# deryrahman/image-caption-emotion-indonesia

Hardware: AMD Instinct MI355X
Metric: images/sec (train step) + NLL loss match, batch=64 ResNet152+FactoredLSTM-512 (higher is better)
Workload: dtype f32 (trunk: operands as 2 f16 pieces each, 3 MFMA products per multiply, f32 accumulate; decoder: large products as 3 bf16 pieces per operand, 6 MFMA products per multiply, the rest f32 MFMA; the persistent LSTM kernel the trunk's split-f16 scheme)

## Files before the change

### image-caption-emotion-indonesia_amd/_lib.py

```python
import ctypes as C
import os

_HERE = os.path.dirname(os.path.abspath(__file__))
LIB_PATH = os.path.join(_HERE, "libcapnet_hip.so")

_f = C.POINTER(C.c_float)
_vp = C.c_void_p
_i = C.c_int
_l = C.c_long
_sz = C.c_size_t
_ip = C.POINTER(C.c_int)

SIGNATURES = {
    "capnet_last_error": (C.c_char_p, []),
    "capnet_abi_version": (_i, []),
    "capnet_sgemm": (_i, [_i, _i, _i, _i, _i, _vp, _l, _vp, _l, _vp, _l, _vp, _i, _i, _l, _l, _l,
                          _l, _i, _vp]),
    "capnet_sgemm_b3": (_i, [_i, _i, _i, _i, _i, _vp, _l, _vp, _l, _vp, _l, _vp, _i, _i, _l, _l, _l, _l, _vp, _sz, _vp]),
    "capnet_sgemm_b3_eligible": (_i, [_i, _i, _i, _i, _i, _vp, _l, _vp, _l, _vp, _l, _vp, _i, _l, _l, _l, _l]),
    "capnet_sgemm_splitk": (_i, [_i, _i, _i, _i, _i, _vp, _l, _vp, _l, _vp, _l, _vp, _i, _vp, _sz, _vp]),
    "capnet_sgemm_splitk_fused": (_i, [_i, _i, _i, _i, _i, _vp, _l, _vp, _l, _vp, _l, _vp, _i, _vp, _sz, _vp, _sz, _vp]),
    "capnet_colsum": (_i, [_vp, _l, _i, _i, _vp, _i, _vp]),
    "capnet_argmax_rows": (_i, [_vp, _i, _i, _i, _vp, _vp]),
    "capnet_resize_u8": (_i, [_vp, _i, _i, _vp, _vp, _i, _i, _vp, _vp, _i, _vp, _vp, _i, _vp]),
# ... 224 lines not shown
                                                                                                  _vp, _vp, _vp]),
    "capnet_beam_nbest": (_i, [_vp, _i, _i, _i, C.c_float, _vp, _vp, _vp, _vp, _vp]),
    "capnet_beam_nbest_traced": (_i, [_vp, _vp, _i, _i, _i, C.c_float, _vp, _vp, _vp, _vp, _vp, _vp]),
    "capnet_beam_decode_ws_beam_offset": (_sz, [_i] * 8),
    "capnet_att_beam_decode_alphas_ws_trace_offset": (_sz, [_i] * 11),
    "capnet_att_beam_decode_alphas_ws_hist_offset": (_sz, [_i] * 11),
    "capnet_alpha_gather": (_i, [_vp, _vp, _i, _i, _i, _i, _vp, _vp]),
    "capnet_lstm_wfrag_floats": (_sz, [_i]),
    "capnet_lstm_pack_wfrag": (_i, [_vp, _vp, _i, _i, _vp]),
    "capnet_lstm_step_fused": (_i, [_vp, _vp, _vp, _l, _vp, _vp, _vp, _i, _i, _i, _vp]),
    "capnet_lstm_step_fused_stamped": (_i, [_vp, _vp, _vp, _l, _vp, _vp, _vp, _i, _i, _vp, _vp]),
    "capnet_lstm_step_fused_supported": (_i, [_i, _i]),
    "capnet_lstm_persist_supported": (_i, [_i, _i]),
    "capnet_lstm_persist_w_floats": (_sz, []),
    "capnet_lstm_persist_ctl_ints": (_sz, []),
    "capnet_lstm_persist_pack": (_i, [_vp, _vp, _i, _vp]),
    "capnet_lstm_persist_run": (_i, [_vp, _vp, _vp, _vp, _ip, _i, _i, _i, _i, _i, _vp, _vp, _vp, _vp]),
    "capnet_xent_fwd": (_i, [_vp, _l, _i, _i, _vp, _vp, _vp, _vp, _vp, _vp]),
    "capnet_xent_bwd": (_i, [_vp, _l, _i, _i, _vp, _vp, _vp, _vp, _l, _vp]),
    "capnet_att_loss_fwd": (_i, [_vp, _vp, _i, _i, _i, C.c_float, _vp, _vp, _vp]),
    "capnet_att_loss_bwd": (_i, [_vp, _vp, _i, _i, _i, C.c_float, _vp, _vp]),
    "capnet_policy_xent_fwd": (_i, [_vp, _l, _i, _i, _vp, _vp, _i, _ip, _i, _vp, _vp, _vp, _vp, _vp, _vp]),
    "capnet_policy_xent_bwd": (_i, [_vp, _l, _i, _i, _vp, _vp, _vp, _i, _ip, _i, _vp, _vp, _l, _vp]),
    "capnet_bleu_rows": (_i, [_vp, _l, _i, _i, C.c_longlong, C.c_longlong, _i, _vp, _vp, _i, _i, _i, C.POINTER(C.c_double), _i,
                              _vp, _vp, _vp]),
    "capnet_cider_rows": (_i, [_vp, _l, _i, _i, C.c_longlong, C.c_longlong, _i, _vp, _vp, _vp, _i, _i, _i, C.POINTER(_vp),
                               C.POINTER(_vp), _ip, C.c_double, C.c_double, _vp, _vp, _vp, _vp]),
    "capnet_clamp_adam": (_i, [_i, C.POINTER(_vp), C.POINTER(_vp), C.POINTER(_vp),
                               C.POINTER(_vp), C.POINTER(_l), _ip, C.c_float, C.c_float,
                               C.c_float, C.c_float, C.c_float, _i, _vp, _vp]),
    "capnet_lstm_persist_set_mode": (_i, [_i]),
    "capnet_att_set_chain_mode": (_i, [_i]),
    "capnet_lstm_pointwise_bwd": (_i, [_vp, _vp, _vp, _vp, _vp, _vp, _i, _i, _i, _vp]),
    "capnet_conv1x1_fwd_areg": (_i, [_vp, _vp, _i, _vp, _vp, _vp, _i, _vp, _vp, _l, _i, _i, _i, _vp]),
    "capnet_trunk_set_timing": (_i, [_vp, _i]),
    "capnet_trunk_time_next_pass": (_i, [_vp]),
    "capnet_trunk_collect_timing": (_i, [_vp, C.POINTER(C.c_double), C.POINTER(_l),
                                         C.POINTER(C.c_double)]),
    "capnet_packed_targets": (_i, [_vp, _i, _i, _ip, _vp, _vp]),
    "capnet_fused_block_weight_words": (_sz, [_i, _i, _i]),
    "capnet_fused_block_pack": (_i, [_vp, _vp, _i, _i, _i, _vp]),
    "capnet_fused_block_stats_floats": (_sz, [_l, _i]),
    "capnet_fused_block_stats": (_i, [_vp, _vp, _vp, _vp, _l, _i, _i, _vp, _vp, _vp, _vp, C.c_float, C.c_float, _vp, _vp, _vp,
                                      _vp, _vp]),
    "capnet_fused_block_tiles": (_i, [_l, _i]),
    "capnet_fused_block_forward": (_i, [_vp] * 14 + [_l, _i, _i, _i, _vp, _vp]),
    "capnet_comm_unique_id": (_i, [_vp]),
    "capnet_comm_create": (_i, [_vp, _i, _i, C.POINTER(_vp)]),
    "capnet_comm_destroy": (_i, [_vp]),
    "capnet_allreduce_grads": (_i, [_vp, _vp, _l, _vp]),
    "capnet_err_word_exchange": (_i, [_vp, _vp, _i, _vp]),
    "capnet_count_skipped": (_i, [_vp, _vp, _vp]),
    "capnet_pack_tensors": (_i, [_i, C.POINTER(_vp), C.POINTER(_l), _vp, _i, C.c_float, _vp]),
    "capnet_clamp": (_i, [_vp, _l, C.c_float, C.c_float, _vp]),
    "capnet_beam_advance_constrained": (_i, [_vp, _vp, _l, _i, _i, _i, _i, _i, C.c_longlong, _i, _i, _vp, _i, _vp, _vp, _vp]),
    "capnet_beam_advance_constrained_traced": (_i, [_vp, _vp, _vp, _l, _i, _i, _i, _i, _i, C.c_longlong, _i, _i, _vp, _i, _vp, _vp,
                                                    _vp]),
    "capnet_beam_topk_banned": (_i, [_vp, _l, _i, _i, _vp, _i, _vp, _i, _vp, _vp, _vp]),
    "capnet_beam_topk_batched_banned": (_i, [_vp, _l, _i, _vp, _vp, _i, _vp, _i, _vp, _vp, _vp]),
    "capnet_beam_decode_constrained": (_i, [_i, _i, _i, _i, _i, _i, _i, _i, C.c_longlong, C.c_longlong, _vp, C.POINTER(_vp),
                                            C.POINTER(_vp), _vp, _vp, _vp, _vp, _vp, _sz, _i, _vp, _vp, C.POINTER(_i), _vp, _vp,
                                            _i, _i, _vp, _i]),
    "capnet_att_beam_decode_constrained": (_i, [_i] * 11 + [C.c_longlong, C.c_longlong] + [_vp] * 7 +
                                           [C.POINTER(_vp), C.POINTER(_vp), _vp, _vp, _vp, _vp, _vp, _sz, _i, _vp, _vp, C.POINTER(_i),
                                            _vp, _vp, _i, _i, _vp, _i]),
    "capnet_att_beam_decode_alphas_constrained": (_i, [_i] * 11 + [C.c_longlong, C.c_longlong] + [_vp] * 7 +
# ... 74 lines not shown
```

### image-caption-emotion-indonesia_amd/csrc/capi.cpp

```cpp
#include "../../include/capnet.h"

#include "common.h"
#include "kernels.h"

using namespace capnet;

static inline hipStream_t S(capnet_stream_t s) { return reinterpret_cast<hipStream_t>(s); }

static SeqDims to_dims(const int* d) {
  SeqDims r;
  r.B = d[0]; r.T = d[1]; r.steps = d[2]; r.N = d[3]; r.E = d[4]; r.F = d[5]; r.H = d[6];
  r.V = d[7]; r.has_features = d[8]; r.cell = d[9];
  return r;
}

static bool weight_used(int cell, int i) { return cell == kCellFactored || i == 0 || i == 4 || i == 24 || i == 28; }
template <class Weights>
static void to_weights(const float* const* weights, Weights& w) {
  for (int g = 0; g < 4; ++g) {
    w.Vw[g] = weights[0 + g];  w.Vb[g] = weights[4 + g];
    w.Sw[g] = weights[8 + g];  w.Sb[g] = weights[12 + g];
    w.Uw[g] = weights[16 + g]; w.Ub[g] = weights[20 + g];
    w.Ww[g] = weights[24 + g]; w.Wb[g] = weights[28 + g];
  }
}
static void to_grads(float* const* q, SeqGrads& g) {
  g.dVcat = q[0]; g.dbV = q[1]; g.dScat = q[2]; g.dbS = q[3]; g.dUcat = q[4];
  g.dbUW = q[5]; g.dWcat = q[6]; g.dEmb = q[7]; g.dFeat = q[8];
}

static AttDims to_adims(const int* d) {
  AttDims r;
  r.B = d[0]; r.T = d[1]; r.steps = d[2]; r.N = d[3]; r.E = d[4]; r.F = d[5]; r.H = d[6];
  r.V = d[7]; r.A = d[8]; r.P = d[9]; r.C = d[10]; r.cell = d[11];
  return r;
}
// ... 1321 lines not shown
                                       const float* Cb, const float* state0, void* workspace, float* slab, size_t slab_floats,
                                       int poll_every, long long* seqs, int* lengths, int* steps_run, int* err_flag,
                                       capnet_stream_t stream, int no_repeat_ngram, int min_words, const int* banned,
                                       int n_banned) {
  const BeamConstraints con{no_repeat_ngram, min_words, banned, n_banned};
  return att_beam_decode_entry(cell, nlayers, 1, n, k, P, A, C, E, H, V, max_steps, start_token, end_token, att1, feat, emb, wz, bz,
                               w_full, b_full, wcat, beff, Cw, Cb, state0, workspace, slab, slab_floats, poll_every, seqs, lengths,
                               steps_run, err_flag, stream, false, nullptr, &con);
}

int capnet_att_beam_decode_alphas_constrained(int cell, int nlayers, int n, int k, int P, int A, int C, int E, int H, int V,
                                              int max_steps, long long start_token, long long end_token,
                                              const float* att1, const float* feat, const float* emb, const float* wz,
                                              const float* bz, const float* w_full, const float* b_full,
                                              const float* const* wcat, const float* const* beff, const float* Cw,
                                              const float* Cb, const float* state0, void* workspace, float* slab,
                                              size_t slab_floats, int poll_every, long long* seqs, int* lengths, int* steps_run,
                                              int* err_flag, capnet_stream_t stream, float* alphas, int no_repeat_ngram,
                                              int min_words, const int* banned, int n_banned) {
  const BeamConstraints con{no_repeat_ngram, min_words, banned, n_banned};
  return att_beam_decode_entry(cell, nlayers, 1, n, k, P, A, C, E, H, V, max_steps, start_token, end_token, att1, feat, emb, wz, bz,
                               w_full, b_full, wcat, beff, Cw, Cb, state0, workspace, slab, slab_floats, poll_every, seqs, lengths,
                               steps_run, err_flag, stream, true, alphas, &con);
}

int capnet_lstm_pointwise_bwd(const float* gates, const float* c, const float* c_prev, const float* dh, float* dc_io,
                              float* dpre, int b, int H, int cell, capnet_stream_t stream) {
  CAPNET_REQUIRE(gates && c && dh && dc_io && dpre && b >= 0 && H > 0, "lstm_pointwise_bwd: bad argument");
  CAPNET_REQUIRE(cell == kCellFactored || cell == kCellLSTM, "lstm_pointwise_bwd: unknown cell %d", cell);
  const bool f = cell == kCellFactored;
  return lstm_pointwise_bwd(gates, 4L * H, c, c_prev, dh, nullptr, dc_io, dpre, 4L * H, b, b, H, 0, 1, f ? 2 : 3, f ? 3 : 2,
                            f ? 0 : 1, S(stream), 0, 0);
}
size_t capnet_lstm_wfrag_floats(int H) { return lstm_wfrag_floats(H); }
int capnet_lstm_pack_wfrag(const float* w_cat, float* w_frag, int H, int cell, capnet_stream_t stream) {
  CAPNET_REQUIRE(cell == kCellFactored || cell == kCellLSTM, "lstm_pack_wfrag: unknown cell %d", cell);
  return cell == kCellFactored ? lstm_pack_wfrag(w_cat, w_frag, H, 0, 1, 2, 3, S(stream))
                               : lstm_pack_wfrag(w_cat, w_frag, H, 0, 1, 3, 2, S(stream));
}
int capnet_lstm_step_fused(const float* h_prev, const float* w_cat, float* gates, long ldg,
                           const float* c_prev, float* c_out, float* h_out, int b, int H, int cell,
                           capnet_stream_t stream) {
  CAPNET_REQUIRE(cell == kCellFactored || cell == kCellLSTM, "lstm_step_fused: unknown cell %d", cell);
  if (cell == kCellFactored)
    return lstm_step_fused(h_prev, w_cat, gates, ldg, c_prev, c_out, h_out, b, H, 0, 1, 2, 3, 0, S(stream));
  return lstm_step_fused(h_prev, w_cat, gates, ldg, c_prev, c_out, h_out, b, H, 0, 1, 3, 2, 1, S(stream));
}
int capnet_lstm_step_fused_stamped(const float* h_prev, const float* w_frag, float* gates, long ldg,
                                   const float* c_prev, float* c_out, float* h_out, int b, int H,
                                   unsigned long long* stamps, capnet_stream_t stream) {
  return lstm_step_fused(h_prev, w_frag, gates, ldg, c_prev, c_out, h_out, b, H, 0, 1, 2, 3, 0,
                         S(stream), stamps);
}
int capnet_lstm_step_fused_supported(int b, int H) { return lstm_step_fused_supported(b, H) ? 1 : 0; }

int capnet_lstm_persist_supported(int b, int H) { return lstm_persist_supported(b, H) ? 1 : 0; }
int capnet_lstm_persist_set_mode(int mode) { return lstm_persist_set_mode(mode); }
size_t capnet_lstm_persist_w_floats(void) { return lstm_persist_w_floats(); }
size_t capnet_lstm_persist_ctl_ints(void) { return lstm_persist_ctl_ints(); }
int capnet_lstm_persist_pack(const float* w_cat, float* w_img, int cell, capnet_stream_t stream) {
  CAPNET_REQUIRE(cell == kCellFactored || cell == kCellLSTM, "lstm_persist_pack: unknown cell %d", cell);
  return cell == kCellFactored ? lstm_persist_pack(w_cat, w_img, 0, 1, 2, 3, S(stream))
                               : lstm_persist_pack(w_cat, w_img, 0, 1, 3, 2, S(stream));
}
int capnet_lstm_persist_run(const float* w_img, float* gates, float* cell_states, float* hiddens,
                            const int* batch_sizes, int t0, int t1, int H, int cell, int segment,
// ... 440 lines not shown
```

### image-caption-emotion-indonesia_amd/csrc/decoder_seq.cpp

```cpp
#include <vector>

#include "common.h"
#include "kernels.h"

#include "seq_layers.h"

namespace capnet {

namespace seqd {

std::vector<int> step_offsets(const int* batch_sizes, int steps) {
  std::vector<int> off(steps + 1, 0);
  for (int t = 0; t < steps; ++t) off[t + 1] = off[t] + batch_sizes[t];
  return off;
}

std::vector<int> with_state_step(int B, const int* batch_sizes, int steps) {
  std::vector<int> bse(steps + 1, B);
  for (int t = 0; t < steps; ++t) bse[t + 1] = batch_sizes[t];
  return bse;
}

int check_batch_sizes(const char* who, const int* batch_sizes, int steps, int B, int N) {
  CAPNET_REQUIRE(batch_sizes != nullptr, "%s: null batch_sizes", who);
// ... 296 lines not shown
      RC(input_chain(c0.d, c0.L, c0.sv, r0, r0 + b, sk, s));
    }
    for (int l = 0; l < nlayers; ++l) {
      LayerCtx& c = lay[l];
      if (l > 0) {
        RC(rows_dropout(lay[l - 1].hid, c.sv + c.L.X, r0, r1, H, dropout_p, seed, l, between_layers(training, dropout_p), s));
        RC(input_chain(c.d, c.L, c.sv, r0, r1, sk, s));
      }
      RC(recur(c, off, batch_sizes, t, t1, skws, skctr, err_flag, s));
    }
    t = t1;
  }
  return kOk;
}

static int seq_backward_layer(const SeqDims& d, const int* batch_sizes, const float* dH, const float* hiddens,
                              const float* saved, const int* saved_i, float* scratch, const SeqGrads& g,
                              float dropout_p, unsigned long long seed, int training, int layer, float* dH_below,
                              hipStream_t s, int lead = 0, float* dh0 = nullptr, float* dc0 = nullptr) {
  RC(check_dims(d, batch_sizes));
  CAPNET_REQUIRE(dH && hiddens && saved && saved_i && scratch, "seq_backward: null argument");
  CAPNET_REQUIRE(g.dWcat && g.dbUW && g.dVcat && (layer > 0 ? dH_below != nullptr : g.dEmb != nullptr), "seq_backward: null gradient buffer");
  CAPNET_REQUIRE(lead == 0 || (layer > 0 && d.steps > 1 && dh0 && dc0), "seq_backward: leading state step");
  const Layout L = make_layout(d);
  const BwdLayout S = make_bwd_layout(d, lead);
  const int E = d.E, F = d.F, H = d.H, N = d.N;
  const bool fac = d.cell == kCellFactored;
  const GateOrder go = gate_order(d.cell);
  const std::vector<int> off = step_offsets(batch_sizes, d.steps);
  const int R0 = off[lead], Nr = N - R0;
  float *dPre = scratch + S.dPre, *Hprev = scratch + S.Hprev, *dh_rec = scratch + S.dh_rec, *dc = scratch + S.dc;
  float *dX = scratch + S.dX, *dA2 = scratch + S.dA2, *dA1 = scratch + S.dA1, *skws = scratch + S.skws;
  const float* sv = saved;
  CAPNET_HIP_CHECK(hipMemsetAsync(dh_rec, 0, (size_t)d.B * H * sizeof(float), s));
  CAPNET_HIP_CHECK(hipMemsetAsync(dc, 0, (size_t)d.B * H * sizeof(float), s));

  int slabs = 0;
  for (int t = d.steps - 1; t >= lead; --t) {
    const int b = batch_sizes[t], r0 = off[t];
    const int b_next = (t + 1 < d.steps) ? batch_sizes[t + 1] : 0;
    RC(lstm_pointwise_bwd(sv + L.G + (size_t)r0 * 4 * H, 4 * H, sv + L.Cst + (size_t)r0 * H,
                          t > 0 ? sv + L.Cst + (size_t)off[t - 1] * H : nullptr,
                          dH + (size_t)(r0 - R0) * H, slabs > 0 ? skws : dh_rec, dc, dPre + (size_t)r0 * 4 * H,
                          4 * H, b, b_next, H, go.gi, go.gf, go.go, go.gg, go.tanh_out, s, slabs,
                          (long)b_next * H));
    slabs = 0;
    if (t > 0) {
      RC(sgemm_splitk_slabs(false, b, H, 4 * H, dPre + (size_t)r0 * 4 * H, 4 * H, sv + L.Wcat, H, skws,
                            kSplitKFloats, &slabs, s));
      if (slabs == 0)
        RC(sgemm_splitk(false, false, b, H, 4 * H, dPre + (size_t)r0 * 4 * H, 4 * H, sv + L.Wcat, H,
                        dh_rec, H, nullptr, 0, skws, kSplitKFloats, s));
    }
  }
  if (lead) {
    if (slabs) RC(reduce_slabs(skws, slabs, batch_sizes[0], H, dh_rec, H, nullptr, 0, s));
    RC(copy_d2d(dh0, dh_rec, (size_t)batch_sizes[0] * H, s));
    RC(copy_d2d(dc0, dc, (size_t)batch_sizes[0] * H, s));
  }
  const float* X = sv + L.X + (size_t)R0 * E;
  const float* A1 = lead ? scratch + S.A1c : sv + L.A1;
  const float* A2 = lead ? scratch + S.A2c : sv + L.A2;
  const Chain ch = chain_of(d, L, sv);
  if (fac && lead) RC(chain_rows(ch, X, Nr, scratch + S.A1c, scratch + S.A2c, SkWs{skws, kSplitKFloats, nullptr}, s));
  dPre += (size_t)R0 * 4 * H;
  RC(gather_rows(hiddens, saved_i + L.prev_row + R0, Hprev, Nr, H, s));
  RC(sgemm_splitk(true, false, 4 * H, H, Nr, dPre, 4 * H, Hprev, H, g.dWcat, H, nullptr, 0, skws, kSplitKFloats, s));
  RC(colsum(dPre, 4 * H, Nr, 4 * H, g.dbUW, 0, s));
  if (fac) {
    CAPNET_REQUIRE(g.dUcat && g.dScat && g.dbS && g.dbV, "seq_backward: null factored gradient buffer");
    RC(chain_bwd_rows(ch, dPre, 4 * H, Nr, dA2, dA1, s));
    RC(chain_wgrads(ch, dPre, 4 * H, X, A1, A2, dA2, dA1, Nr, ChainGrads{g.dVcat, g.dbV, g.dScat, g.dbS, g.dUcat}, s));
  } else {
    RC(lstm_input_wgrad(dPre, 4 * H, X, E, H, Nr, g.dVcat, s));
  }
  const int K = fac ? 4 * F : 4 * H;
  RC(sgemm_splitk(false, false, Nr, E, K, fac ? dA1 : dPre, K, sv + L.Vcat, E, dX, E, nullptr, 0, skws, kSplitKFloats, s));
  if (layer > 0) return rows_dropout(dX, dH_below, 0, Nr, E, dropout_p, seed, layer, between_layers(training, dropout_p), s);
  CAPNET_HIP_CHECK(hipMemsetAsync(g.dEmb, 0, (size_t)d.V * E * sizeof(float), s));
  if (g.dFeat) CAPNET_HIP_CHECK(hipMemsetAsync(g.dFeat, 0, (size_t)d.B * E * sizeof(float), s));
  return scatter_input_grad(dX, E, N, E, saved_i + L.row_sample, saved_i + L.row_col, saved_i + L.row_token, g.dEmb, g.dFeat, d.V,
                            dropout_p, seed, training && dropout_p > 0.f, s, reinterpret_cast<int*>(skws), kSplitKFloats);
}

int seqd::seq_backward_upper(const SeqDims& d, const int* batch_sizes, const float* dH, const float* hiddens,
                             const float* saved, const int* saved_i, float* scratch, const SeqGrads& g, float dropout_p,
                             unsigned long long seed, int training, int layer, float* dH_below, float* dh0, float* dc0,
                             hipStream_t s) {
  return seq_backward_layer(d, batch_sizes, dH, hiddens, saved, saved_i, scratch, g, dropout_p, seed, training, layer,
// ... 22 lines not shown
```

### image-caption-emotion-indonesia_amd/csrc/kernels.h

```cpp
#pragma once
#include <hip/hip_runtime.h>

namespace capnet {

int sgemm(bool ta, bool tb, int M, int N, int K, const float* A, long lda, const float* B,
          long ldb, float* C, long ldc, const float* bias, int accumulate, int batch, long sA,
          long sB, long sC, long sBias, int force_tile, hipStream_t stream);

bool sgemm_b3_eligible(bool ta, bool tb, int M, int N, int K, const float* A, long lda, const float* B, long ldb,
                       const float* C, long ldc, const float* bias, int batch, long sA, long sB, long sC, long sBias);
int sgemm_b3(bool ta, bool tb, int M, int N, int K, const float* A, long lda, const float* B, long ldb, float* C, long ldc,
             const float* bias, int accumulate, int batch, long sA, long sB, long sC, long sBias, hipStream_t stream,
             float* ws = nullptr, size_t ws_floats = 0);

constexpr size_t kSplitKCounters = 1024;
int sgemm_splitk(bool ta, bool tb, int M, int N, int K, const float* A, long lda, const float* B,
                 long ldb, float* C, long ldc, const float* bias, int accumulate, float* ws,
                 size_t ws_floats, hipStream_t stream, int* counters = nullptr, size_t n_counters = 0);
int sgemm_splitk_slabs(bool tb, int M, int N, int K, const float* A, long lda, const float* B, long ldb,
                       float* ws, size_t ws_floats, int* n_slabs, hipStream_t stream);
int sgemm_rows16_slabs(bool tb, int M, int N, int K, const float* A, long lda, const float* B, long ldb, float* ws,
                       size_t ws_floats, int* n_slabs, hipStream_t stream);
int sgemm_splitk_batched(bool ta, bool tb, int M, int N, int K, const float* A, long lda,
                         const float* B, long ldb, float* C, long ldc, const float* bias,
// ... 123 lines not shown
  int off[kMaxSteps + 1];
  unsigned char tf[kMaxSteps];
};
int build_rows(const SeqMeta& m, int* row_sample, int* row_col, int* row_token, int* prev_row,
               hipStream_t stream);
int gather_inputs(const long long* captions, int T, const float* features, const float* emb, int E,
                  int V, const int* row_sample, const int* row_col, int* row_token, float* X,
                  long ldx, int r0, int r1, float p, unsigned long long seed, int use_dropout,
                  int dynamic, int* err_flag, hipStream_t stream);
int embedding_fwd(const long long* idx, int n, const float* emb, int E, int V, float* out,
                  int* err_flag, hipStream_t stream);
int packed_targets(const SeqMeta& m, const long long* captions, int T, long long* out,
                   hipStream_t stream);
struct CopyTable {
  static constexpr int kMax = 40;
  const float* src[kMax];
  const float* src2[kMax];
  float* dst[kMax];
  size_t n[kMax];
  int count = 0;
  void add(float* d, const float* a, size_t len, const float* b = nullptr) {
    if (count < kMax) { src[count] = a; src2[count] = b; dst[count] = d; n[count] = len; }
    ++count;
  }
};
int multi_copy(const CopyTable& t, hipStream_t stream);
int lstm_pointwise_fwd(float* pre, long ldp, const float* c_prev, float* c_out, float* h_out, int b,
                       int H, int gi, int gf, int go, int gg, int tanh_out, hipStream_t stream,
                       const float* slabs = nullptr, int n_slabs = 0);
int lstm_pointwise_bwd(const float* gates, long ldg, const float* c, const float* c_prev,
                       const float* dH, const float* dh_rec, float* dc_io, float* dpre, long ldq,
                       int b, int b_next, int H, int gi, int gf, int go, int gg, int tanh_out,
                       hipStream_t stream, int dh_slabs = 0, long dh_slab_stride = 0);
int gather_prev_rows(const float* src, const int* idx, const float* first, const int* sample,
                     float* out, int rows, int C, hipStream_t stream);
int argmax_rows(const float* x, int rows, int ld, int V, int* out, hipStream_t stream);
int beam_topk(const float* logits, long ld, int rows, int V, const float* prev, int k,
              float* out_scores, long long* out_index, hipStream_t stream);
int beam_topk_banned(float* logits, long ld, int rows, int V, const float* prev, int k, const int* bans, int cap,
                     float* out_scores, long long* out_index, hipStream_t stream);
size_t beam_state_bytes(int n, int k, int max_steps);
int beam_init(void* beam, int n, int k, int max_steps, long long start_token, long long* prev_words, hipStream_t stream);
struct BeamConstraints {
  int no_repeat_ngram, min_words;
  const int* banned;
  int n_banned;
  const int* forced = nullptr;
  int n_forced = 0;
};
struct BeamTeams {
  int teams;
  float strength;
  void* beam;
};
int beam_constraints_check(const char* who, const BeamConstraints& c);
int beam_forced_check(const char* who, const BeamConstraints& c);
int beam_teams_check(const char* who, int k, int teams, float strength);
int beam_advance(const char* who, void* beam, float* logits, long ld, int V, int n, int k, int max_steps, int step,
                 long long end_token, const BeamConstraints* con, const BeamTeams* teams, long long* next_words,
                 long long* parent_rows, void* trace, hipStream_t stream);
int beam_topk_batched(const char* who, float* logits, long ld, int V, const float* prev, const int* meta, int n, const int* bans,
                      int cap, const BeamTeams* teams, const int* met, const int* forced, int n_forced, long long end_token,
                      float* out_scores, long long* out_index, hipStream_t stream);
size_t beam_trace_bytes(int n, int k, int max_steps);
int beam_advance_topk(void* beam, const float* values, const int* index, const float* lse, int V, int n, int k, int max_steps,
                      int step, long long end_token, long long* next_words, long long* parent_rows, hipStream_t stream);
// ... 328 lines not shown
```

### image-caption-emotion-indonesia_amd/csrc/seq_kernels.hip

```cpp
#include "common.h"
#include "dropout_mask.h"
#include "kernels.h"
#include "step_core.h"

namespace capnet {

__global__ __launch_bounds__(256) void build_rows_kernel(SeqMeta m, int* __restrict__ row_sample,
                                                         int* __restrict__ row_col,
                                                         int* __restrict__ row_token,
                                                         int* __restrict__ prev_row) {
  const int r = blockIdx.x * blockDim.x + threadIdx.x;
  if (r >= m.N) return;
  int t = 0;
  while (t + 1 < m.steps && r >= m.off[t + 1]) ++t;
  const int j = r - m.off[t];
  row_sample[r] = j;
  row_token[r] = -1;
  prev_row[r] = t > 0 ? m.off[t - 1] + j : -1;
  int col;
  if (m.tf[t]) col = m.has_features ? (t == 0 ? -1 : t - 1) : t;
  else col = (t == 0) ? -3 : -2;
  row_col[r] = col;
}

// ... 186 lines not shown
    const float* __restrict__ gates, long ldg, const float* __restrict__ c,
    const float* __restrict__ c_prev, const float* __restrict__ dH,
    const float* __restrict__ dh_rec, float* __restrict__ dc_io, float* __restrict__ dpre, long ldq,
    int b, int b_next, int H, int gi, int gf, int go, int gg, int tanh_out, int dh_slabs,
    long dh_slab_stride) {
  const int idx = blockIdx.x * blockDim.x + threadIdx.x;
  if (idx >= b * H) return;
  const int row = idx / H, j = idx - row * H;
  const float* p = gates + (long)row * ldg;
  const float i = p[gi * H + j], f = p[gf * H + j], o = p[go * H + j], g = p[gg * H + j];
  const float ct = c[(long)row * H + j];
  const float cp = c_prev ? c_prev[(long)row * H + j] : 0.f;
  float dh = dH[(long)row * H + j];
  float dc = 0.f;
  if (row < b_next) {
    if (dh_slabs > 0) {
      const float* sp = dh_rec + (long)row * H + j;
      float s = 0.f;
      int k = 0;
      for (; k + 8 <= dh_slabs; k += 8) {
        float v[8];
#pragma unroll
        for (int u = 0; u < 8; ++u) v[u] = sp[(long)(k + u) * dh_slab_stride];
#pragma unroll
        for (int u = 0; u < 8; ++u) s += v[u];
      }
      for (; k < dh_slabs; ++k) s += sp[(long)k * dh_slab_stride];
      dh += s;
    } else if (dh_rec) {
      dh += dh_rec[(long)row * H + j];
    }
    dc = dc_io[(long)row * H + j];
  }
  float d_o;
  if (tanh_out) {
    const float tc = tanhf(ct);
    d_o = dh * tc;
    dc += dh * o * (1.f - tc * tc);
  } else {
    d_o = dh * ct;
    dc += dh * o;
  }
  const float di = dc * g, dg = dc * i, df = dc * cp;
  float* q = dpre + (long)row * ldq;
  q[gi * H + j] = di * i * (1.f - i);
  q[gf * H + j] = df * f * (1.f - f);
  q[go * H + j] = d_o * o * (1.f - o);
  q[gg * H + j] = dg * (1.f - g * g);
  dc_io[(long)row * H + j] = dc * f;
}

int lstm_pointwise_bwd(const float* gates, long ldg, const float* c, const float* c_prev,
                       const float* dH, const float* dh_rec, float* dc_io, float* dpre, long ldq,
                       int b, int b_next, int H, int gi, int gf, int go, int gg, int tanh_out,
                       hipStream_t stream, int dh_slabs, long dh_slab_stride) {
  if (b <= 0) return kOk;
  hipLaunchKernelGGL(lstm_pointwise_bwd_kernel, dim3(cdiv((long)b * H, 256)), dim3(256), 0, stream,
                     gates, ldg, c, c_prev, dH, dh_rec, dc_io, dpre, ldq, b, b_next, H, gi, gf, go,
                     gg, tanh_out, dh_slabs, dh_slab_stride);
  CAPNET_LAUNCH_CHECK();
  return kOk;
}

__global__ __launch_bounds__(256) void argmax_rows_kernel(const float* __restrict__ x, int ld,
                                                          int V, int* __restrict__ out) {
  const int row = blockIdx.x;
  const float* p = x + (long)row * ld;
  float best = -INFINITY;
  int bi = 0x7fffffff;
  int done = 0;
  if (ld % 4 == 0 && (reinterpret_cast<size_t>(x) & 15) == 0) {
    const int V4 = V / 4;
    for (int j0 = threadIdx.x; j0 < V4; j0 += 8 * 256) {
      float4 v[8];
#pragma unroll
      for (int u = 0; u < 8; ++u) v[u] = *reinterpret_cast<const float4*>(p + 4 * (long)min(j0 + 256 * u, V4 - 1));
#pragma unroll
      for (int u = 0; u < 8; ++u) {
        const int j = 4 * (j0 + 256 * u);
        if (j0 + 256 * u < V4) {
          if (v[u].x > best) { best = v[u].x; bi = j; }
          if (v[u].y > best) { best = v[u].y; bi = j + 1; }
// ... 265 lines not shown
```

### image-caption-emotion-indonesia_amd/csrc/step_core.h

```cpp
#pragma once
#include <hip/hip_runtime.h>
#include <type_traits>

namespace capnet {

typedef float f32x4 __attribute__((ext_vector_type(4)));
__host__ __device__ __forceinline__ int clamp_row(int r, int n) { return r < n ? r : n - 1; }

template <int NJ>
__device__ __forceinline__ f32x4 mfma_chain(const f32x4 (&av)[NJ], const f32x4 (&wv)[NJ], f32x4 acc) {
#pragma unroll
  for (int j = 0; j < NJ; ++j)
#pragma unroll
    for (int e = 0; e < 4; ++e) acc = __builtin_amdgcn_mfma_f32_16x16x4f32(av[j][e], wv[j][e], acc, 0, 0, 0);
  return acc;
}
template <int WAVES, int ROWS>
__device__ __forceinline__ float sum_partials(const float (*red)[ROWS][17], int row, int col, float init) {
  float s = init;
#pragma unroll
  for (int w = 0; w < WAVES; ++w) s += red[w][row][col];
  return s;
}

__device__ __forceinline__ float sigm(float x) { return 1.f / (1.f + expf(-x)); }

__device__ __forceinline__ void lstm_cell(float pi, float pf, float po, float pg, float cp, float& i, float& f, float& o,
                                          float& g, float& c) {
  i = sigm(pi), f = sigm(pf), o = sigm(po), g = tanhf(pg);
  c = f * cp + i * g;
}
__device__ __forceinline__ float lstm_cell_h(float o, float c, int tanh_out) { return tanh_out ? o * tanhf(c) : o * c; }

constexpr bool step_hidden_supported(int H) { return H == 64 || H == 128 || H == 256 || H == 512 || H == 1024; }
template <int N> using nj_t = std::integral_constant<int, N>;
template <class F>
static inline void dispatch_nj(int H, F&& f) {
  switch (H) {
    case 64: f(nj_t<1>{}); break;
    case 128: f(nj_t<2>{}); break;
    case 256: f(nj_t<4>{}); break;
    case 512: f(nj_t<8>{}); break;
    default: f(nj_t<16>{}); break;
  }
}

}
```

### include/capnet.h

```cpp
#ifndef CAPNET_H_
#define CAPNET_H_

#include <stddef.h>

#ifdef __cplusplus
extern "C" {
#endif

typedef void* capnet_stream_t;
typedef struct capnet_trunk capnet_trunk_t;

#define CAPNET_OK 0
#define CAPNET_ERR_INVALID_ARG (-1)
#define CAPNET_ERR_HIP (-2)

const char* capnet_last_error(void);
int capnet_abi_version(void);

int capnet_sgemm(int transA, int transB, int M, int N, int K, const float* A, long lda,
                 const float* B, long ldb, float* C, long ldc, const float* bias, int accumulate,
                 int batch, long strideA, long strideB, long strideC, long strideBias,
                 int force_tile, capnet_stream_t stream);
int capnet_sgemm_b3(int transA, int transB, int M, int N, int K, const float* A, long lda, const float* B, long ldb,
                    float* C, long ldc, const float* bias, int accumulate, int batch, long strideA, long strideB,
// ... 199 lines not shown
                           const long long* captions, const float* features, const float* emb,
                           const float* const* weights, const float* Cw, const float* Cb,
                           float dropout_p, unsigned long long seed, int training, float* saved,
                           int* saved_i, float* scratch, float* hiddens, float* alphas,
                           int* err_flag, capnet_stream_t stream);
int capnet_att_seq_backward(const int* dims, const int* batch_sizes, const float* d_hiddens,
                            const float* d_alphas, const float* hiddens, const float* features,
                            const float* const* weights, const float* saved, const int* saved_i,
                            float* scratch, float* const* grads, float dropout_p,
                            unsigned long long seed, int training, capnet_stream_t stream);

size_t capnet_att_stacked_saved_floats(const int* dims, int layer);
size_t capnet_att_stacked_saved_ints(const int* dims, int layer);
size_t capnet_att_stacked_fwd_scratch_floats(const int* dims, int nlayers);
size_t capnet_att_stacked_bwd_scratch_floats(const int* dims, int nlayers);
int capnet_att_seq_forward_stacked(const int* dims, int nlayers, const int* batch_sizes, const unsigned char* tf_mask,
                                   const long long* captions, const float* features, const float* emb,
                                   const float* const* weights, const float* Cw, const float* Cb, float dropout_p,
                                   unsigned long long seed, int training, float* const* saved, int* const* saved_i,
                                   float* scratch, float* const* hiddens, float* alphas, int* err_flag,
                                   capnet_stream_t stream);
int capnet_att_seq_backward_stacked(const int* dims, int nlayers, const int* batch_sizes, const float* d_hiddens,
                                    const float* d_alphas, const float* const* hiddens, const float* features,
                                    const float* const* weights, const float* const* saved, const int* const* saved_i,
                                    float* scratch, float* const* dh_work, float* const* grads, float dropout_p,
                                    unsigned long long seed, int training, capnet_stream_t stream);

int capnet_embedding_fwd(const long long* idx, int n, const float* emb, int E, int V, float* out,
                         int* err_flag, capnet_stream_t stream);
int capnet_lstm_pointwise_fwd(float* pre, const float* c_prev, float* c_out, float* h_out, int b,
                              int H, int cell, capnet_stream_t stream);
int capnet_lstm_pointwise_bwd(const float* gates, const float* c, const float* c_prev, const float* dh, float* dc_io,
                              float* dpre, int b, int H, int cell, capnet_stream_t stream);

int capnet_stacked_decode_step(int nlayers, int rows, int E, int H, int V, const long long* tokens, const float* x,
                               const float* const* wcat, const float* const* beff, const float* state_in,
                               float* state_out, float* h_top, int* err_flag, capnet_stream_t stream);

int capnet_stacked_decode_step_cell(int cell, int nlayers, int rows, int E, int H, int V, const long long* tokens,
                                    const float* x, const float* const* wcat, const float* const* beff,
                                    const float* state_in, float* state_out, float* h_top, int* err_flag,
                                    capnet_stream_t stream);

int capnet_stacked_decode_step_gather(int cell, int nlayers, int rows, int E, int H, int V, const long long* tokens,
                                      const float* x, const float* const* wcat, const float* const* beff,
                                      const float* state_in, const long long* parent_rows, float* state_out, float* h_top,
                                      int* err_flag, capnet_stream_t stream);

int capnet_stacked_decode_step_groups(int cell, int nlayers, int groups, int rows_per_group, int E, int H, int V,
                                      const long long* tokens, const float* x, const float* const* wcat,
                                      const float* const* beff, const float* state_in, const long long* parent_rows,
                                      float* state_out, float* h_top, int* err_flag, capnet_stream_t stream);

int capnet_stacked_decode_step_tables(int cell, int nlayers, int groups, int rows_per_group, int E, int H, int V,
                                      const long long* tokens, const float* const* tables, const float* const* wcat,
                                      const float* const* beff, const float* state_in, const long long* parent_rows,
                                      float* state_out, float* h_top, int* err_flag, capnet_stream_t stream);

size_t capnet_vocab_argmax_ws_bytes(int rows, int V);
int capnet_vocab_argmax(const float* h, const float* w, const float* b, int rows, int H, int V, void* workspace,
                        long long* tokens, capnet_stream_t stream);

size_t capnet_vocab_argmax_groups_ws_bytes(int groups, int rows_per_group, int V);
int capnet_vocab_argmax_groups(const float* h, const float* const* w, const float* const* b, int groups, int rows_per_group,
                               int H, int V, void* workspace, long long* tokens, capnet_stream_t stream);

// ... 447 lines not shown
```

Measured before the change: 9137.

## Fuse LSTM BPTT pointwise backward with recurrent dh product into one kernel

Adds a single-launch kernel per backward timestep that reduces the incoming split-K slabs, computes the LSTM cell gradients, stages the gate gradients in shared memory, and multiplies them against the recurrent weights with f32 MFMA, writing per-block partial slabs. This replaces a pointwise-backward launch plus a separate split-K sgemm per step, cutting launches and global round-trips on the latency-bound sequential recurrence. Ping-pong slab buffers avoid read/write conflicts between steps, and an environment variable can disable the path. The trade-offs are more slab partials to reduce (H/8 of them) and plain f32 MFMA where the old GEMM may have used a different precision scheme.

```diff
diff --git a/image-caption-emotion-indonesia_amd/_lib.py b/image-caption-emotion-indonesia_amd/_lib.py
--- a/image-caption-emotion-indonesia_amd/_lib.py
+++ b/image-caption-emotion-indonesia_amd/_lib.py
@@ -280,6 +280,7 @@
     "capnet_lstm_persist_set_mode": (_i, [_i]),
     "capnet_att_set_chain_mode": (_i, [_i]),
     "capnet_lstm_pointwise_bwd": (_i, [_vp, _vp, _vp, _vp, _vp, _vp, _i, _i, _i, _vp]),
+    "capnet_lstm_bptt_step": (_i, [_vp, _vp, _vp, _vp, _vp, _i, _vp, _vp, _i, _i, _i, _i, _vp, _vp, _sz, _ip, _i, _vp]),
     "capnet_conv1x1_fwd_areg": (_i, [_vp, _vp, _i, _vp, _vp, _vp, _i, _vp, _vp, _l, _i, _i, _i, _vp]),
     "capnet_trunk_set_timing": (_i, [_vp, _i]),
     "capnet_trunk_time_next_pass": (_i, [_vp]),
diff --git a/image-caption-emotion-indonesia_amd/csrc/capi.cpp b/image-caption-emotion-indonesia_amd/csrc/capi.cpp
--- a/image-caption-emotion-indonesia_amd/csrc/capi.cpp
+++ b/image-caption-emotion-indonesia_amd/csrc/capi.cpp
@@ -2,6 +2,8 @@
 
 #include "common.h"
 #include "kernels.h"
+#include "seq_layers.h"
+#include "step_core.h"
 
 using namespace capnet;
 
@@ -1389,6 +1391,29 @@
   return lstm_pointwise_bwd(gates, 4L * H, c, c_prev, dh, nullptr, dc_io, dpre, 4L * H, b, b, H, 0, 1, f ? 2 : 3, f ? 3 : 2,
                             f ? 0 : 1, S(stream), 0, 0);
 }
+int capnet_lstm_bptt_step(const float* gates, const float* c, const float* c_prev, const float* dh, const float* slabs_in,
+                          int n_in, float* dc_io, float* dpre, int b, int b_next, int H, int cell, const float* w_cat,
+                          float* slabs_out, size_t slab_floats, int* n_out, int fused, capnet_stream_t stream) {
+  CAPNET_REQUIRE(gates && c && dh && dc_io && dpre && n_out && b > 0 && H > 0 && b_next >= 0 && b_next <= b && n_in >= 0 &&
+                     (n_in == 0 || slabs_in) && (!w_cat || slabs_out),
+                 "lstm_bptt_step: bad argument");
+  CAPNET_REQUIRE(cell == kCellFactored || cell == kCellLSTM, "lstm_bptt_step: unknown cell %d", cell);
+  const seqd::GateOrder go = seqd::gate_order(cell);
+  *n_out = 0;
+  if (fused) {
+    CAPNET_REQUIRE(b <= 64 && step_hidden_supported(H), "lstm_bptt_step: b=%d H=%d has no one-launch form", b, H);
+    const int n = w_cat ? lstm_bptt_step_slabs(H) : 0;
+    CAPNET_REQUIRE((size_t)n * b * H <= slab_floats, "lstm_bptt_step: %d slabs need %zu floats", n, (size_t)n * b * H);
+    RC(lstm_bptt_step(gates, 4L * H, c, c_prev, dh, slabs_in, n_in, dc_io, dpre, 4L * H, b, b_next, H, go.gi, go.gf, go.go, go.gg,
+                      go.tanh_out, w_cat, slabs_out, S(stream)));
+    *n_out = n;
+    return kOk;
+  }
+  RC(lstm_pointwise_bwd(gates, 4L * H, c, c_prev, dh, n_in > 0 ? slabs_in : nullptr, dc_io, dpre, 4L * H, b, b_next, H, go.gi, go.gf,
+                        go.go, go.gg, go.tanh_out, S(stream), n_in, (long)b_next * H));
+  if (!w_cat) return kOk;
+  return sgemm_splitk_slabs(false, b, H, 4 * H, dpre, 4L * H, w_cat, H, slabs_out, slab_floats, n_out, S(stream));
+}
 size_t capnet_lstm_wfrag_floats(int H) { return lstm_wfrag_floats(H); }
 int capnet_lstm_pack_wfrag(const float* w_cat, float* w_frag, int H, int cell, capnet_stream_t stream) {
   CAPNET_REQUIRE(cell == kCellFactored || cell == kCellLSTM, "lstm_pack_wfrag: unknown cell %d", cell);
diff --git a/image-caption-emotion-indonesia_amd/csrc/decoder_seq.cpp b/image-caption-emotion-indonesia_amd/csrc/decoder_seq.cpp
--- a/image-caption-emotion-indonesia_amd/csrc/decoder_seq.cpp
+++ b/image-caption-emotion-indonesia_amd/csrc/decoder_seq.cpp
@@ -352,13 +352,27 @@
   float *dPre = scratch + S.dPre, *Hprev = scratch + S.Hprev, *dh_rec = scratch + S.dh_rec, *dc = scratch + S.dc;
   float *dX = scratch + S.dX, *dA2 = scratch + S.dA2, *dA1 = scratch + S.dA1, *skws = scratch + S.skws;
   const float* sv = saved;
-  CAPNET_HIP_CHECK(hipMemsetAsync(dh_rec, 0, (size_t)d.B * H * sizeof(float), s));
+  const bool fused = lstm_bptt_step_supported(batch_sizes[0], H) && aligned16(dH) && aligned16(sv + L.G) && aligned16(sv + L.Cst) &&
+                     aligned16(sv + L.Wcat) && aligned16(scratch);
+  const int fslabs = fused ? lstm_bptt_step_slabs(H) : 0;
+  float* area[2] = {skws, skws + (size_t)fslabs * batch_sizes[0] * H};
+  if (!fused) CAPNET_HIP_CHECK(hipMemsetAsync(dh_rec, 0, (size_t)d.B * H * sizeof(float), s));
   CAPNET_HIP_CHECK(hipMemsetAsync(dc, 0, (size_t)d.B * H * sizeof(float), s));
 
   int slabs = 0;
+  const float* slab_area = skws;
   for (int t = d.steps - 1; t >= lead; --t) {
     const int b = batch_sizes[t], r0 = off[t];
     const int b_next = (t + 1 < d.steps) ? batch_sizes[t + 1] : 0;
+    if (fused) {
+      RC(lstm_bptt_step(sv + L.G + (size_t)r0 * 4 * H, 4 * H, sv + L.Cst + (size_t)r0 * H,
+                        t > 0 ? sv + L.Cst + (size_t)off[t - 1] * H : nullptr, dH + (size_t)(r0 - R0) * H, area[(t + 1) & 1], slabs,
+                        dc, dPre + (size_t)r0 * 4 * H, 4 * H, b, b_next, H, go.gi, go.gf, go.go, go.gg, go.tanh_out,
+                        t > 0 ? sv + L.Wcat : nullptr, area[t & 1], s));
+      slabs = t > 0 ? fslabs : 0;
+      slab_area = area[t & 1];
+      continue;
+    }
     RC(lstm_pointwise_bwd(sv + L.G + (size_t)r0 * 4 * H, 4 * H, sv + L.Cst + (size_t)r0 * H,
                           t > 0 ? sv + L.Cst + (size_t)off[t - 1] * H : nullptr,
                           dH + (size_t)(r0 - R0) * H, slabs > 0 ? skws : dh_rec, dc, dPre + (size_t)r0 * 4 * H,
@@ -374,7 +388,7 @@
     }
   }
   if (lead) {
-    if (slabs) RC(reduce_slabs(skws, slabs, batch_sizes[0], H, dh_rec, H, nullptr, 0, s));
+    if (slabs) RC(reduce_slabs(slab_area, slabs, batch_sizes[0], H, dh_rec, H, nullptr, 0, s));
     RC(copy_d2d(dh0, dh_rec, (size_t)batch_sizes[0] * H, s));
     RC(copy_d2d(dc0, dc, (size_t)batch_sizes[0] * H, s));
   }
diff --git a/image-caption-emotion-indonesia_amd/csrc/kernels.h b/image-caption-emotion-indonesia_amd/csrc/kernels.h
--- a/image-caption-emotion-indonesia_amd/csrc/kernels.h
+++ b/image-caption-emotion-indonesia_amd/csrc/kernels.h
@@ -179,6 +179,11 @@
                        const float* dH, const float* dh_rec, float* dc_io, float* dpre, long ldq,
                        int b, int b_next, int H, int gi, int gf, int go, int gg, int tanh_out,
                        hipStream_t stream, int dh_slabs = 0, long dh_slab_stride = 0);
+bool lstm_bptt_step_supported(int b0, int H);
+int lstm_bptt_step_slabs(int H);
+int lstm_bptt_step(const float* gates, long ldg, const float* c, const float* c_prev, const float* dH, const float* slabs_in,
+                   int n_in, float* dc_io, float* dpre, long ldq, int b, int b_next, int H, int gi, int gf, int go, int gg,
+                   int tanh_out, const float* W, float* slabs_out, hipStream_t stream);
 int gather_prev_rows(const float* src, const int* idx, const float* first, const int* sample,
                      float* out, int rows, int C, hipStream_t stream);
 int argmax_rows(const float* x, int rows, int ld, int V, int* out, hipStream_t stream);
diff --git a/image-caption-emotion-indonesia_amd/csrc/lstm_bptt_step.hip b/image-caption-emotion-indonesia_amd/csrc/lstm_bptt_step.hip
--- /dev/null
+++ b/image-caption-emotion-indonesia_amd/csrc/lstm_bptt_step.hip
@@ -0,0 +1,155 @@
+#include "common.h"
+#include "kernels.h"
+#include "mfma_core.h"
+#include "seq_layers.h"
+#include "step_core.h"
+
+namespace capnet {
+
+namespace {
+
+typedef float f32x2 __attribute__((ext_vector_type(2)));
+
+constexpr int kBpttThreads = 512;
+constexpr int kBpttRows = 64;
+constexpr int kBpttLda = 65;
+constexpr int kBpttDepth = 32;
+constexpr int kBpttUS = 8;
+
+struct BpttArgs {
+  const float *gates, *c, *c_prev, *dH, *slabs_in, *W;
+  float *dc_io, *dpre, *slabs_out;
+  long ldg, ldq;
+  int b, b_next, H, n_in, gi, gf, go, gg, tanh_out;
+};
+
+template <int US>
+__global__ __launch_bounds__(kBpttThreads) __attribute__((amdgpu_waves_per_eu(4))) void lstm_bptt_step_kernel(const BpttArgs a) {
+  constexpr int K = 4 * US, KS = K / 2;
+  __shared__ float sA[K * kBpttLda];
+  const int tid = threadIdx.x, lane = tid & 63, wave = tid >> 6, li = lane & 31, lh = lane >> 5;
+  const int H = a.H, b = a.b, j0 = blockIdx.x * US, ncg = H >> 6;
+  const bool prod = a.W != nullptr;
+
+  f32x2 w[KS];
+  auto load_w = [&](int cg) {
+#pragma unroll
+    for (int ks = 0; ks < KS; ++ks) {
+      const int kl = 2 * ks + lh;
+      const long wrow = (long)(kl / US) * H + j0 + kl % US;
+      w[ks] = *reinterpret_cast<const f32x2*>(a.W + wrow * H + cg * 64 + 2 * li);
+    }
+  };
+  if (prod && wave < ncg) load_w(wave);
+
+  for (int it = tid; it < b * US; it += kBpttThreads) {
+    const int row = it / US, ul = it - row * US, j = j0 + ul;
+    const long off = (long)row * H + j;
+    const float* p = a.gates + (long)row * a.ldg + j;
+    const float i = p[(long)a.gi * H], f = p[(long)a.gf * H], o = p[(long)a.go * H], g = p[(long)a.gg * H];
+    const float ct = a.c[off], cp = a.c_prev ? a.c_prev[off] : 0.f;
+    float dh = a.dH[off], dc = 0.f;
+    if (row < a.b_next) {
+      if (a.n_in > 0) {
+        const unsigned stride = (unsigned)a.b_next * H, so = (unsigned)off;
+        float s = 0.f;
+        for (int k = 0; k < a.n_in; k += kBpttDepth) {
+          float v[kBpttDepth];
+#pragma unroll
+          for (int q = 0; q < kBpttDepth; ++q) v[q] = a.slabs_in[so + (unsigned)min(k + q, a.n_in - 1) * stride];
+#pragma unroll
+          for (int q = 0; q < kBpttDepth; ++q)
+            if (k + q < a.n_in) s += v[q];
+        }
+        dh += s;
+      }
+      dc = a.dc_io[off];
+    }
+    float dpi, dpf, dpo, dpg, dcp;
+    lstm_cell_bwd(i, f, o, g, ct, cp, dh, dc, a.tanh_out, dpi, dpf, dpo, dpg, dcp);
+    float* q = a.dpre + (long)row * a.ldq + j;
+    q[(long)a.gi * H] = dpi;
+    q[(long)a.gf * H] = dpf;
+    q[(long)a.go * H] = dpo;
+    q[(long)a.gg * H] = dpg;
+    a.dc_io[off] = dcp;
+    if (prod) {
+      sA[(a.gi * US + ul) * kBpttLda + row] = dpi;
+      sA[(a.gf * US + ul) * kBpttLda + row] = dpf;
+      sA[(a.go * US + ul) * kBpttLda + row] = dpo;
+      sA[(a.gg * US + ul) * kBpttLda + row] = dpg;
+    }
+  }
+  if (!prod) return;
+  const int nrt = (b + 31) >> 5, pad = 32 * nrt - b;
+  for (int it = tid; it < K * pad; it += kBpttThreads) sA[(it / pad) * kBpttLda + b + it % pad] = 0.f;
+  __syncthreads();
+
+  auto product = [&](int cg) {
+    for (int rt = 0; rt < nrt; ++rt) {
+      f32x16 acc0, acc1;
+#pragma unroll
+      for (int r = 0; r < 16; ++r) acc0[r] = 0.f, acc1[r] = 0.f;
+      const float* ap = sA + lh * kBpttLda + rt * 32 + li;
+#pragma unroll
+      for (int ks = 0; ks < KS; ++ks) {
+        const float av = ap[2 * ks * kBpttLda];
+        acc0 = __builtin_amdgcn_mfma_f32_32x32x2f32(av, w[ks][0], acc0, 0, 0, 0);
+        acc1 = __builtin_amdgcn_mfma_f32_32x32x2f32(av, w[ks][1], acc1, 0, 0, 0);
+      }
+      float* out = a.slabs_out + (long)blockIdx.x * b * H + cg * 64 + 2 * li;
+#pragma unroll
+      for (int r = 0; r < 16; ++r) {
+        const int m = rt * 32 + (r & 3) + 8 * (r >> 2) + 4 * lh;
+        if (m < b) {
+          const f32x2 v = {acc0[r], acc1[r]};
+          *reinterpret_cast<f32x2*>(out + (long)m * H) = v;
+        }
+      }
+    }
+  };
+  if (wave < ncg) product(wave);
+  if (wave + 8 < ncg) {
+    load_w(wave + 8);
+    product(wave + 8);
+  }
+}
+
+bool bptt_disabled() {
+  static const bool off = [] { const char* e = getenv("CAPNET_NO_FUSED_BPTT"); return e && e[0] == '1'; }();
+  return off;
+}
+
+}
+
+int lstm_bptt_step_slabs(int H) { return H / kBpttUS; }
+
+bool lstm_bptt_step_supported(int b0, int H) {
+  return !bptt_disabled() && b0 > 0 && b0 <= kBpttRows && step_hidden_supported(H) &&
+         2 * (size_t)lstm_bptt_step_slabs(H) * b0 * H <= kSplitKFloats;
+}
+
+int lstm_bptt_step(const float* gates, long ldg, const float* c, const float* c_prev, const float* dH, const float* slabs_in,
+                   int n_in, float* dc_io, float* dpre, long ldq, int b, int b_next, int H, int gi, int gf, int go, int gg,
+                   int tanh_out, const float* W, float* slabs_out, hipStream_t stream) {
+  if (b <= 0) return kOk;
+  CAPNET_REQUIRE(b <= kBpttRows && b_next >= 0 && b_next <= b && step_hidden_supported(H), "lstm_bptt_step: b=%d b_next=%d H=%d", b, b_next, H);
+  CAPNET_REQUIRE(gates && c && dH && dc_io && dpre && (!W || slabs_out) && (n_in == 0 || (slabs_in && n_in == lstm_bptt_step_slabs(H))),
+                 "lstm_bptt_step: bad argument");
+  CAPNET_REQUIRE(ldg % 4 == 0 && ldq % 4 == 0 && aligned16(gates) && aligned16(c) && (!c_prev || aligned16(c_prev)) && aligned16(dH) &&
+                     (!slabs_in || aligned16(slabs_in)) && aligned16(dc_io) && aligned16(dpre) && (!W || (aligned16(W) && aligned16(slabs_out))),
+                 "lstm_bptt_step: 16-byte alignment");
+  CAPNET_REQUIRE((unsigned)gi < 4 && (unsigned)gf < 4 && (unsigned)go < 4 && (unsigned)gg < 4 && ((1 << gi) | (1 << gf) | (1 << go) | (1 << gg)) == 15,
+                 "lstm_bptt_step: gate order");
+  BpttArgs a;
+  a.gates = gates; a.c = c; a.c_prev = c_prev; a.dH = dH; a.slabs_in = slabs_in; a.W = W;
+  a.dc_io = dc_io; a.dpre = dpre; a.slabs_out = slabs_out;
+  a.ldg = ldg; a.ldq = ldq;
+  a.b = b; a.b_next = b_next; a.H = H; a.n_in = b_next > 0 ? n_in : 0;
+  a.gi = gi; a.gf = gf; a.go = go; a.gg = gg; a.tanh_out = tanh_out;
+  hipLaunchKernelGGL(lstm_bptt_step_kernel<kBpttUS>, dim3(H / kBpttUS), dim3(kBpttThreads), 0, stream, a);
+  CAPNET_LAUNCH_CHECK();
+  return kOk;
+}
+
+}
diff --git a/image-caption-emotion-indonesia_amd/csrc/seq_kernels.hip b/image-caption-emotion-indonesia_amd/csrc/seq_kernels.hip
--- a/image-caption-emotion-indonesia_amd/csrc/seq_kernels.hip
+++ b/image-caption-emotion-indonesia_amd/csrc/seq_kernels.hip
@@ -242,22 +242,14 @@
     }
     dc = dc_io[(long)row * H + j];
   }
-  float d_o;
-  if (tanh_out) {
-    const float tc = tanhf(ct);
-    d_o = dh * tc;
-    dc += dh * o * (1.f - tc * tc);
-  } else {
-    d_o = dh * ct;
-    dc += dh * o;
-  }
-  const float di = dc * g, dg = dc * i, df = dc * cp;
+  float dpi, dpf, dpo, dpg, dc_prev;
+  lstm_cell_bwd(i, f, o, g, ct, cp, dh, dc, tanh_out, dpi, dpf, dpo, dpg, dc_prev);
   float* q = dpre + (long)row * ldq;
-  q[gi * H + j] = di * i * (1.f - i);
-  q[gf * H + j] = df * f * (1.f - f);
-  q[go * H + j] = d_o * o * (1.f - o);
-  q[gg * H + j] = dg * (1.f - g * g);
-  dc_io[(long)row * H + j] = dc * f;
+  q[gi * H + j] = dpi;
+  q[gf * H + j] = dpf;
+  q[go * H + j] = dpo;
+  q[gg * H + j] = dpg;
+  dc_io[(long)row * H + j] = dc_prev;
 }
 
 int lstm_pointwise_bwd(const float* gates, long ldg, const float* c, const float* c_prev,
diff --git a/image-caption-emotion-indonesia_amd/csrc/step_core.h b/image-caption-emotion-indonesia_amd/csrc/step_core.h
--- a/image-caption-emotion-indonesia_amd/csrc/step_core.h
+++ b/image-caption-emotion-indonesia_amd/csrc/step_core.h
@@ -32,6 +32,25 @@
 }
 __device__ __forceinline__ float lstm_cell_h(float o, float c, int tanh_out) { return tanh_out ? o * tanhf(c) : o * c; }
 
+__device__ __forceinline__ void lstm_cell_bwd(float i, float f, float o, float g, float ct, float cp, float dh, float dc,
+                                              int tanh_out, float& dpi, float& dpf, float& dpo, float& dpg, float& dc_prev) {
+  float d_o;
+  if (tanh_out) {
+    const float tc = tanhf(ct);
+    d_o = dh * tc;
+    dc += dh * o * (1.f - tc * tc);
+  } else {
+    d_o = dh * ct;
+    dc += dh * o;
+  }
+  const float di = dc * g, dg = dc * i, df = dc * cp;
+  dpi = di * i * (1.f - i);
+  dpf = df * f * (1.f - f);
+  dpo = d_o * o * (1.f - o);
+  dpg = dg * (1.f - g * g);
+  dc_prev = dc * f;
+}
+
 constexpr bool step_hidden_supported(int H) { return H == 64 || H == 128 || H == 256 || H == 512 || H == 1024; }
 template <int N> using nj_t = std::integral_constant<int, N>;
 template <class F>
diff --git a/include/capnet.h b/include/capnet.h
--- a/include/capnet.h
+++ b/include/capnet.h
@@ -255,6 +255,9 @@
                               int H, int cell, capnet_stream_t stream);
 int capnet_lstm_pointwise_bwd(const float* gates, const float* c, const float* c_prev, const float* dh, float* dc_io,
                               float* dpre, int b, int H, int cell, capnet_stream_t stream);
+int capnet_lstm_bptt_step(const float* gates, const float* c, const float* c_prev, const float* dh, const float* slabs_in,
+                          int n_in, float* dc_io, float* dpre, int b, int b_next, int H, int cell, const float* w_cat,
+                          float* slabs_out, size_t slab_floats, int* n_out, int fused, capnet_stream_t stream);
 
 int capnet_stacked_decode_step(int nlayers, int rows, int E, int H, int V, const long long* tokens, const float* x,
                                const float* const* wcat, const float* const* beff, const float* state_in,
```

New measurement: 9125. Within noise of the previous version (-0.1%).
